# ebiggers/libdeflate

Measured on NVIDIA H100. Metric: MB/s compress+decompress (batched 64 KiB chunks), higher is better.
Workload: dtype u8

## Files before the change

### libdeflate_b200/csrc/deflate_kernel.cu

```cuda
#include "ldb_common.cuh"

#define DEF_THREADS 256

__global__ void __launch_bounds__(DEF_THREADS)
ldb_deflate_stored_kernel(ldb_deflate_args a)
{
	for (size_t c = blockIdx.x; c < a.n; c += gridDim.x) {
		const u8 *in = (const u8 *)a.in_ptrs[c];
		const size_t n = a.in_nbytes[c];
		u8 *out = (u8 *)a.out_ptrs[c];
		const size_t avail = a.out_avail[c];
		const u32 overhead = a.format == LDB_FMT_GZIP ? 18 : (a.format == LDB_FMT_ZLIB ? 6 : 0);
		const u32 hdr = a.format == LDB_FMT_GZIP ? 10 : (a.format == LDB_FMT_ZLIB ? 2 : 0);
		const size_t nblocks = n ? (n + 65534) / 65535 : 1;
		const size_t need = n + 5 * nblocks;
		bool fits = !(overhead && avail <= overhead) && need <= avail - overhead;
		if (!fits) {
			if (threadIdx.x == 0) a.out_nbytes[c] = 0;
			continue;
		}
		if (threadIdx.x == 0) def_write_header(out, a.format, a.level);
		const bool final_piece = !(a.piece && (a.piece[c] & LDB_PIECE_NONFINAL));
		u8 *dst = out + hdr;
		for (size_t b = 0; b < nblocks; b++) {
			size_t off = b * 65535;
			u32 len = (u32)(n - off > 65535 ? 65535 : n - off);
			if (threadIdx.x == 0) {
				dst[0] = (b + 1 == nblocks && final_piece) ? 1 : 0;
				dst[1] = (u8)len; dst[2] = (u8)(len >> 8);
				dst[3] = (u8)~len; dst[4] = (u8)(~len >> 8);
			}
			for (u32 i = threadIdx.x; i < len; i += DEF_THREADS) dst[5 + i] = in[off + i];
			dst += 5 + len;
		}
		if (threadIdx.x == 0) {
			u32 t = def_write_trailer(dst, a.format, a.checksums ? a.checksums[c] : 0, n);
			a.out_nbytes[c] = (size_t)(dst - out) + t;
		}
	}
}

#include "deflate_lz_kernel.cuh"

int ldb_deflate_grid(const ldb_launch_cfg &cfg) { return cfg.num_sms; }

int ldb_launch_deflate(const ldb_deflate_args &a, const ldb_launch_cfg &cfg, void *stream)
{
	if (a.n == 0) return 0;
	if (a.level == 0) {
		size_t blocks = a.n < (size_t)cfg.num_sms * 8 ? a.n : (size_t)cfg.num_sms * 8;
		LDB_LAUNCH(ldb_deflate_stored_kernel, dim3((unsigned)blocks), dim3(DEF_THREADS), 0, (cudaStream_t)stream, a);
		LDB_CUDA_CHECK_RET(cudaGetLastError());
		return 0;
	}
	return ldb_launch_deflate_lz(a, cfg, stream);
}
```

### libdeflate_b200/csrc/deflate_lz_kernel.cuh

```cuda
#pragma once

#ifndef LZ_THREADS
#define LZ_THREADS   1024
#endif
#define LZ_WARPS     (LZ_THREADS / 32)
#define LZ_PASS      16384
#define LZ_BLOCK_PASSES 2
#define LZ_NWIN      (LZ_PASS / 32)
#define LZ_NSL_BITS  (LZ_WARPS >= 32 ? 5 : 4)
#define LZ_NSL       (1 << LZ_NSL_BITS)
#ifndef LZ_QUANTUM
#define LZ_QUANTUM   0
#endif
#define LZ_SEG       16384
#define LZ_RING      65536
#define LZ_HASH_BITS 13
#define LZ_WIN       32768
#define LZ_LOOKAHEAD 512
#define LZ_MAX_DIST  (LZ_WIN - LZ_LOOKAHEAD)
#define LZ_TOKCAP    (LZ_BLOCK_PASSES * LZ_PASS + 64)
#define LZ_STAGE_WORDS 2048
#define LZ_TPT(gt)     ((gt) > 512 ? 1u : 2u)
#ifndef LZ_PWARPS
#define LZ_PWARPS    12
#endif
#define LZ_BAR_P     1
#ifndef LZ_PF
#define LZ_PF        4
#endif
#ifndef LZ_SPEC_ROUNDS
#define LZ_SPEC_ROUNDS 4
#endif
static_assert(LZ_SPEC_ROUNDS >= 1 && LZ_SPEC_ROUNDS <= 14, "round statistic buckets");
static_assert(LZ_PWARPS >= 10 && LZ_PWARPS < LZ_WARPS, "parse/flush group: 320..LZ_THREADS-32 threads");

#define LZ_SM_RING   0
#define LZ_SM_NEXT   (LZ_SM_RING + LZ_RING)
#define LZ_SM_HEAD   (LZ_SM_NEXT + 2 * 65536)
#define LZ_SM_R      (LZ_SM_HEAD + 2 * (1 << LZ_HASH_BITS))
#define LZ_SM_VIS    (LZ_SM_R)
#define LZ_SM_TOKOFF (LZ_SM_R + 4096)
#define LZ_SM_ENTRY  (LZ_SM_R + 8320)
#define LZ_SM_ESCAN  (LZ_SM_R + 9344)
#define LZ_SM_GEXIT  (LZ_SM_R + 9728)
#define LZ_SM_ITEMS  (LZ_SM_R + 12288)
#define LZ_SM_FREQ   (LZ_SM_ITEMS + 1024)
#define LZ_SM_LENS   (LZ_SM_FREQ + 4 * 320)
#define LZ_SM_CODES  (LZ_SM_LENS + 320)
#define LZ_SM_VARS   (LZ_SM_CODES + 2 * 320)
// ... 15 lines not shown
	u32 chunk;
	u32 tok_count;
	u32 parse_entry;
	u32 cost_dyn, cost_static, extra_bits;
	u32 hlit, hdist, hclen;
	u32 n_items;
	u32 run_counter;
	u32 min_len;
	u32 far4_dist;
	u32 used_lits[8];
	u32 carry;
	u32 nused_lit, nused_off;
	u32 huff_over;
	u32 obs_blk[8], obs_next[8];
	u32 end_early;
	u32 failed;
	u32 obit_lo, obit_hi;
	u32 blk_begin, blk_entry, blk_passes;
	u32 pre_lens_packed[3];
	u32 tma_phase;
	u32 dict, nonfinal;
	u32 spec_last;
	u32 spec_first;
};
static_assert(sizeof(lz_vars) <= 256, "lz_vars fits its shared-memory slot");

struct lz_params {
	int depth, nice, lazy;
	int opt_iters;
};

__device__ __forceinline__ lz_params lz_level_params(int level)
{
	switch (level) {
	case 1: return {2, 16, 0, 0};
	case 2: return {4, 24, 0, 0};
	case 3: return {8, 32, 0, 0};
	case 4: return {12, 48, 0, 0};
	case 5: return {12, 48, 1, 0};
#ifndef LZ_L6_DEPTH
#define LZ_L6_DEPTH 24
#endif
	case 6: return {LZ_L6_DEPTH, 96, 1, 0};
	case 7: return {48, 160, 1, 0};
	case 8: return {96, 258, 2, 0};
	case 9: return {200, 258, 2, 0};
// ... 10 lines not shown
	else if (num_used_literals < 8) m = 8;
	else if (num_used_literals < 10) m = 7;
	else if (num_used_literals < 16) m = 6;
	else if (num_used_literals < 45) m = 5;
	else m = 4;
	if (depth < 16) {
		u32 cap = depth < 5 ? 4 : (depth < 10 ? 5 : 7);
		if (m > cap) m = cap;
	}
	return m;
}

__device__ __forceinline__ u32 lz_ld32(const u8 *ring, u32 pos)
{
	u32 a = pos & (LZ_RING - 1);
	const u32 *w = (const u32 *)ring;
	u32 lo = w[a >> 2];
	u32 hi = w[((a + 4) & (LZ_RING - 1)) >> 2];
	return __funnelshift_r(lo, hi, (a & 3) * 8);
}
__device__ __forceinline__ u32 lz_ld8(const u8 *ring, u32 pos) { return ring[pos & (LZ_RING - 1)]; }
__device__ __forceinline__ u32 lz_hash(u32 v) { return (v * 0x1E35A7BDu) >> (32 - LZ_HASH_BITS); }

__device__ __forceinline__ void lz_load_segment(u8 *sm, lz_vars *v, const u8 *in, u32 from, u32 to)
{
	u8 *ring = sm + LZ_SM_RING;
	u32 len = to - from;
	u32 bulk = (((uintptr_t)(in + from) & 15) == 0) ? (len & ~15u) : 0;
	__syncthreads();
#ifndef LDB_EMU
	if (bulk) {
		u32 mbar = (u32)__cvta_generic_to_shared(&v->mbar);
		if (threadIdx.x == 0) {
			u32 dst = (u32)__cvta_generic_to_shared(ring + (from & (LZ_RING - 1)));
			asm volatile("fence.proxy.async.shared::cta;" ::: "memory");
			asm volatile("mbarrier.arrive.expect_tx.shared::cta.b64 _, [%0], %1;" ::"r"(mbar), "r"(bulk) : "memory");
			asm volatile("cp.async.bulk.shared::cluster.global.mbarrier::complete_tx::bytes [%0], [%1], %2, [%3];"
				     ::"r"(dst), "l"(in + from), "r"(bulk), "r"(mbar) : "memory");
		}
		u32 phase = v->tma_phase;
		u32 done = 0;
		while (!done) {
			asm volatile("{\n\t.reg .pred p;\n\tmbarrier.try_wait.parity.shared::cta.b64 p, [%1], %2;\n\tselp.u32 %0, 1, 0, p;\n\t}"
				     : "=r"(done) : "r"(mbar), "r"(phase) : "memory");
		}
	}
#else
	for (u32 i = threadIdx.x; i < bulk; i += LZ_THREADS) ring[(from + i) & (LZ_RING - 1)] = in[from + i];
#endif
	for (u32 i = bulk + threadIdx.x; i < len; i += LZ_THREADS) ring[(from + i) & (LZ_RING - 1)] = in[from + i];
	__syncthreads();
	if (bulk && threadIdx.x == 0) v->tma_phase ^= 1;
	__syncthreads();
}

__device__ __forceinline__ u32 lz_len_slot(u32 len)
{
	if (len < 11) return len - 3;
	if (len == 258) return 28;
	u32 l = len - 3;
	u32 eb = 29 - __clz(l);
	return 4 * eb + 4 + ((l >> eb) & 3);
}
__device__ __forceinline__ u32 lz_len_extra_bits(u32 slot) { return (slot < 8 || slot == 28) ? 0 : (slot - 4) >> 2; }
__device__ __forceinline__ u32 lz_len_base(u32 slot) { return slot < 8 ? 3 + slot : (slot == 28 ? 258 : 3 + ((4 + (slot & 3)) << ((slot - 4) >> 2))); }
__device__ __forceinline__ u32 lz_off_slot(u32 off)
{
	if (off < 5) return off - 1;
	u32 o = off - 1;
	u32 eb = 30 - __clz(o);
	return 2 * eb + 2 + ((o >> eb) & 1);
}
__device__ __forceinline__ u32 lz_off_extra_bits(u32 slot) { return slot < 4 ? 0 : (slot - 2) >> 1; }
__device__ __forceinline__ u32 lz_off_base(u32 slot) { return slot < 4 ? 1 + slot : 1 + ((2 + (slot & 1)) << ((slot - 2) >> 1)); }

__device__ __forceinline__ u32 lz_static_litlen_len(u32 sym) { return sym < 144 ? 8 : (sym < 256 ? 9 : (sym < 280 ? 7 : 8)); }
// ... 50 lines not shown
	}
}

__device__ __forceinline__ void lz_gen_codes_serial(const u8 *lens, u32 nsyms, u16 *codes)
{
	u32 cnt[16];
	for (u32 l = 0; l < 16; l++) cnt[l] = 0;
	for (u32 s = 0; s < nsyms; s++) cnt[lens[s]]++;
	u32 next[16];
	u32 code = 0;
	cnt[0] = 0;
	for (u32 l = 1; l < 16; l++) {
		next[l] = code;
		code = (code + cnt[l]) << 1;
	}
	for (u32 s = 0; s < nsyms; s++) {
		u32 l = lens[s];
		codes[s] = l ? (u16)(__brev(next[l]++) >> (32 - l)) : 0;
	}
}

#ifdef LZ_TIMING
#include <stdio.h>
__device__ unsigned long long ldb_lz_timing[2][16];
#define LZ_T(k) do { if (tid == 0 || tid == 32 * LZ_PWARPS) { long long t_ = clock64(); tacc[k] += t_ - tlast; tlast = t_; } } while (0)
#else
#define LZ_T(k) do { } while (0)
#endif

#ifdef LZ_SPEC_STATS
__device__ unsigned long long ldb_lz_spec_rounds[16];
extern "C" __attribute__((visibility("default"))) void ldb_lz_spec_stats(unsigned long long *out, int reset)
{
#ifdef LDB_EMU
	for (int i = 0; i < 16; i++) { out[i] = ldb_lz_spec_rounds[i]; if (reset) ldb_lz_spec_rounds[i] = 0; }
#else
	unsigned long long z[16] = {};
	cudaDeviceSynchronize();
	cudaMemcpyFromSymbol(out, ldb_lz_spec_rounds, sizeof(z));
	if (reset) cudaMemcpyToSymbol(ldb_lz_spec_rounds, z, sizeof(z));
#endif
}
#endif

template <int NBITS>
__device__ __forceinline__ u32 lz_same_key_mask(u32 key, bool valid)
{
	u32 m = __ballot_sync(LDB_FULL_MASK, valid);
#pragma unroll
	for (int b = 0; b < NBITS; b++) {
		const u32 bal = __ballot_sync(LDB_FULL_MASK, (key >> b) & 1);
		m &= ((key >> b) & 1) ? bal : ~bal;
	}
	return m;
}

__device__ __forceinline__ void lz_insert_pass_par(const u8 *ring, u16 *head, u16 *nextt, u32 *cmat,
						   u32 b0, u32 pend, u32 n, u32 tid, u32 lane, u32 warp
#ifdef LZ_TIMING
						   , long long *tacc, long long &tlast
#endif
						   )
{
	static_assert(LZ_WARPS >= LZ_NSL && (LZ_WARPS * LZ_NSL + 2 * LZ_NSL) * 4 <= 8192, "one linking warp per slice");
	u32 *sbase = cmat + LZ_WARPS * LZ_NSL, *stot = sbase + LZ_NSL;
	const u32 lt = (1u << lane) - 1;
	const u32 LB = (b0 + LZ_PASS) & 0xffff;
	const u32 ntiles = (pend - b0 + 31) >> 5, tpw = (ntiles + LZ_WARPS - 1) / LZ_WARPS;
	const u32 r0 = b0 + warp * tpw * 32;
	const u32 r1 = r0 + tpw * 32 < pend ? r0 + tpw * 32 : pend;
	for (u32 i = tid; i < LZ_WARPS * LZ_NSL + 2 * LZ_NSL; i += LZ_THREADS) cmat[i] = 0;
	__syncthreads();
	for (u32 p = r0 + lane; p < r1; p += 32) {
		const u32 hv = p + 4 <= n ? lz_hash(lz_ld32(ring, p)) : 0xffffu;
		nextt[p & 0xffff] = (u16)hv;
		if (hv != 0xffffu) atomicAdd(&cmat[warp * LZ_NSL + (hv >> (LZ_HASH_BITS - LZ_NSL_BITS))], 1u);
	}
	__syncthreads();
	LZ_T(12);
	if (warp == 0) {
		u32 run = 0;
		if (lane < LZ_NSL)
			for (u32 w = 0; w < LZ_WARPS; w++) {
				const u32 c = cmat[w * LZ_NSL + lane];
				cmat[w * LZ_NSL + lane] = run;
				run += c;
			}
		u32 incl = run;
		for (int o2 = 1; o2 < LZ_NSL; o2 <<= 1) {
			const u32 t = __shfl_up_sync(LDB_FULL_MASK, incl, o2);
			if (lane >= (u32)o2) incl += t;
		}
		if (lane < LZ_NSL) { sbase[lane] = incl - run; stot[lane] = run; }
	}
	__syncthreads();
	for (u32 t = 0; t < tpw; t++) {
		const u32 p = r0 + 32 * t + lane;
		const u32 hv = p < r1 ? nextt[p & 0xffff] : 0xffffu;
		const bool valid = hv != 0xffffu;
		const u32 sl = hv >> (LZ_HASH_BITS - LZ_NSL_BITS);
		const u32 m = lz_same_key_mask<LZ_NSL_BITS>(sl, valid);
		const u32 cur = valid ? cmat[warp * LZ_NSL + sl] : 0;
		__syncwarp();
		if (valid) {
			nextt[LB + sbase[sl] + cur + __popc(m & lt)] = (u16)p;
			if ((m & lt) == 0) cmat[warp * LZ_NSL + sl] = cur + __popc(m);
		}
		__syncwarp();
	}
	__syncthreads();
	LZ_T(13);
	if (warp < LZ_NSL) {
		const u32 cnt = stot[warp];
		const u16 *mylist = nextt + LB + sbase[warp];
		u32 p16n = lane < cnt ? mylist[lane] : 0;
		u32 hn = lane < cnt ? nextt[p16n] : 0;
		for (u32 b = 0; b < cnt; b += 32) {
			const bool valid = b + lane < cnt;
			const u32 p16 = p16n;
			const u32 h = valid ? hn : 0;
			if (b + 32 + lane < cnt) {
				p16n = mylist[b + 32 + lane];
				hn = nextt[p16n];
			}
			const u32 old_head = valid ? head[h] : 0;
			const u32 m = lz_same_key_mask<LZ_HASH_BITS - LZ_NSL_BITS>(h, valid);
			const u32 below = m & lt;
			const u32 prev = __shfl_sync(LDB_FULL_MASK, p16, below ? 31 - __clz(below) : 0);
			if (valid) {
				nextt[p16] = (u16)(below ? prev : old_head);
				if ((m >> lane) == 1) head[h] = (u16)p16;
			}
			__syncwarp();
		}
	}
	__syncthreads();
}

__device__ __forceinline__ void lz_search(const u8 *ring, const u16 *nextt, u32 p, u32 n, int depth, u32 nice_level,
					   u32 &best_len, u32 &best_dist)
{
	const u32 max_len = n - p < 258 ? n - p : 258;
	const u32 nice = nice_level < max_len ? nice_level : max_len;
	if (best_len) {
		while (best_len < max_len && lz_ld8(ring, p + best_len) == lz_ld8(ring, p - best_dist + best_len)) best_len++;
	}
	if (best_len >= nice) return;
	const u32 cur = lz_ld32(ring, p);
	u32 tailo = best_len >= 4 ? best_len - 3 : 0;
	u32 tailv = tailo ? lz_ld32(ring, p + tailo) : cur;
	const u32 lim = p < LZ_MAX_DIST ? p : LZ_MAX_DIST;
	u32 cand = nextt[p & 0xffff];
	u32 prev_dist = 0;
	for (int d = 0; d < depth; d++) {
		const u32 dist = (p - cand) & 0xffff;
		if (dist - 1 >= lim || dist <= prev_dist) break;
		prev_dist = dist;
		const u32 cq = cand;
		cand = nextt[cq];
// ... 244 lines not shown
	u32 *escan = (u32 *)(sm + LZ_SM_ESCAN);
	u16 *gexit = (u16 *)(sm + LZ_SM_GEXIT);
	u32 *freq = (u32 *)(sm + LZ_SM_FREQ);
	u8 *lens = sm + LZ_SM_LENS;
	u16 *codes = (u16 *)(sm + LZ_SM_CODES);
	lz_vars *v = (lz_vars *)(sm + LZ_SM_VARS);
	u32 *stage = (u32 *)(sm + LZ_SM_R);
	u16 *hsorted = (u16 *)(sm + LZ_SM_R);
	u32 *hnodefreq = (u32 *)(sm + LZ_SM_R + 1024);
	u16 *hparent = (u16 *)(sm + LZ_SM_R + 1024 + 2304);
	u16 *osorted = (u16 *)(sm + LZ_SM_R + 4608);
	u32 *onodefreq = (u32 *)(sm + LZ_SM_R + 4608 + 128);
	u16 *oparent = (u16 *)(sm + LZ_SM_R + 4608 + 128 + 512);
	u16 *items = (u16 *)(sm + LZ_SM_ITEMS);
	u8 *gs = a.scratch + 256 + (size_t)blockIdx.x * LZ_GS_BYTES;
	u32 *res = (u32 *)(gs + LZ_GS_RES);
	u32 *tokbuf = (u32 *)(gs + LZ_GS_TOK);
	u32 *costg = (u32 *)(gs + LZ_GS_COST);
	u32 *mlist = (u32 *)(gs + LZ_GS_MLIST);
	u8 *costtab = sm + LZ_SM_ITEMS;

	const u32 tid = threadIdx.x, lane = tid & 31, warp = tid >> 5;
#ifdef LZ_TIMING
	long long tacc[16] = {};
	long long tlast = clock64();
#endif
	const lz_params P = lz_level_params(a.level);
	const bool pipe = !P.opt_iters;
	u32 GW = LZ_WARPS, GT = LZ_THREADS;
	auto gsync = [&]() {
		if (GT < LZ_THREADS) LDB_BAR_SYNC(LZ_BAR_P, GT);
		else __syncthreads();
	};

	if (tid == 0) {
		v->tma_phase = 0;
#ifndef LDB_EMU
		u32 mbar = (u32)__cvta_generic_to_shared(&v->mbar);
		asm volatile("mbarrier.init.shared::cta.b64 [%0], 1;" ::"r"(mbar) : "memory");
		asm volatile("fence.mbarrier_init.release.cluster;" ::: "memory");
#endif
	}
	__syncthreads();

	for (;;) {
		if (tid == 0) v->chunk = atomicAdd(a.work_counter, 1u);
		__syncthreads();
		const size_t c = v->chunk;
		__syncthreads();
		if (c >= a.n) break;

		const u32 pflags = PIECES ? a.piece[c] : 0;
		const u32 dict = pflags & LDB_PIECE_DICT_MASK;
		const bool final_piece = !(pflags & LDB_PIECE_NONFINAL);
		const u8 *in = (const u8 *)a.in_ptrs[c];
		const size_t n64 = a.in_nbytes[c];
		lz_out o;
		o.out = (u8 *)a.out_ptrs[c];
		o.avail = a.out_avail[c];
		o.obit = 0;
		const u32 overhead = a.format == LDB_FMT_GZIP ? 18 : (a.format == LDB_FMT_ZLIB ? 6 : 0);
		const u32 trailer = a.format == LDB_FMT_GZIP ? 8 : (a.format == LDB_FMT_ZLIB ? 4 : 0);
		const u32 hdr_bytes = overhead - trailer;

		const bool passthrough = n64 <= (size_t)(55 - 4 * a.level) || n64 > 0x7fff0000u;
		bool fits = !(overhead && o.avail <= overhead);
		if (passthrough || !fits) {
			const size_t nblocks = n64 ? (n64 + 65534) / 65535 : 1;
			fits = fits && (n64 + 5 * nblocks <= o.avail - overhead);
			if (!fits) {
				if (tid == 0) a.out_nbytes[c] = 0;
				continue;
			}
			if (tid == 0) def_write_header(o.out, a.format, a.level);
			u8 *dst = o.out + hdr_bytes;
			for (size_t b = 0; b < nblocks; b++) {
				size_t off = b * 65535;
				u32 len = (u32)(n64 - off > 65535 ? 65535 : n64 - off);
				if (tid == 0) {
					dst[0] = (b + 1 == nblocks && final_piece) ? 1 : 0;
					dst[1] = (u8)len; dst[2] = (u8)(len >> 8);
					dst[3] = (u8)~len; dst[4] = (u8)(~len >> 8);
				}
				for (u32 i = tid; i < len; i += LZ_THREADS) dst[5 + i] = in[off + i];
				dst += 5 + len;
			}
			if (tid == 0) {
				u32 t = def_write_trailer(dst, a.format, a.checksums ? a.checksums[c] : 0, n64);
				a.out_nbytes[c] = (size_t)(dst - o.out) + t;
			}
			continue;
		}
		const u32 n = (u32)n64 + dict;
		in -= dict;

		for (u32 i = tid; i < (1u << LZ_HASH_BITS) / 2; i += LZ_THREADS) ((u32 *)head)[i] = 0xffffffffu;
		if (tid == 0) {
			v->failed = 0;
			v->parse_entry = dict;
			if (PIECES) { v->dict = dict; v->nonfinal = !final_piece; }
			v->tok_count = 0;
			u8 h[12] = {0, 0, 0, 0, 0, 0, 0, 0, 0, 0, 0, 0};
			def_write_header(h, a.format, a.level);
			u32 whole = hdr_bytes & ~3u;
			for (u32 i = 0; i < whole; i++) o.out[i] = h[i];
			u32 cw = 0;
			for (u32 i = whole; i < hdr_bytes; i++) cw |= (u32)h[i] << (8 * (i - whole));
			v->carry = cw;
		}
		for (u32 i = tid; i < 320; i += LZ_THREADS) freq[i] = 0;
		o.obit = (u64)hdr_bytes * 8;
		__syncthreads();

		auto parse_pass = [&](const u32 pb0, const u32 ppend, const u32 aoff, const bool forced, u16 *exitt) {
			const u32 nwin = (ppend - pb0 + 31) >> 5;
			const u32 min_len = v->min_len, far4 = v->far4_dist;
			const u32 G = (nwin + GW - 1) / GW;
			const u32 wbeg = warp * G, wend = wbeg + G < nwin ? wbeg + G : nwin;
			auto res_load = [&](u32 w) -> u32 {
				const u32 i = w * 32 + lane;
// ... 266 lines not shown
				for (u32 l = 15; l >= 1; l--) {
					cum += cn[l];
					if (myrank < cum) { len = l; break; }
				}
				lens[tid] = (u8)len;
			}
			gsync();
			if (tid < 320) {
				const u32 l = lens[tid];
				u32 code = 0;
				if (l) {
					const u32 *cn = is_lit ? hcount : ocount;
					u32 first = 0;
					for (u32 k = 1; k < l; k++) first = (first + cn[k]) << 1;
					u32 same = 0;
					for (u32 t = lo; t < tid; t++) same += lens[t] == l;
					code = __brev(first + same) >> (32 - l);
				}
				codes[tid] = (u16)code;
			}
			gsync();
		};

		u32 loaded_end = 0;
		u32 block_begin = dict;
		u32 block_entry = dict;
		u32 pass_in_block = 0;

		auto search_pass = [&](const u32 b0, const u32 pend, u32 *rs) {
			const u32 min_len = v->min_len, far4 = v->far4_dist;
#ifndef LZ_RUN_SHORT
#define LZ_RUN_SHORT 16
#endif
			const u32 run_len = a.level >= 7 ? 32 : LZ_RUN_SHORT;
			u32 i = 0, i_end = 0;
			u32 pL = 0, pD = 0;
			u32 pending = 0;
#if LZ_QUANTUM
			lz_walk wk;
			wk.left = 0; wk.best_len = 0; wk.best_dist = 0; wk.cand = 0; wk.prev_dist = 0; wk.tailo = 0; wk.tailv = 0; wk.cur = 0;
			bool in_search = false;
#endif
			for (;;) {
#if LZ_QUANTUM
				if (!in_search) {
#endif
				if (i >= i_end || b0 + i >= pend) {
					const u32 r = atomicAdd(&v->run_counter, 1u);
					i = r * run_len;
					if (b0 + i >= pend || i >= LZ_PASS) break;
					i_end = i + run_len;
					pending = 0;
				}
#if LZ_QUANTUM
					const u32 p0 = b0 + i;
					wk.best_len = 0; wk.best_dist = 0; wk.left = 0;
					if (p0 + 4 <= n) {
						u32 sL = 0, sD = 0;
						if (pending) { sL = pL - pending >= 4 ? pL - pending : 0; sD = pD; }
						lz_walk_setup(ring, nextt, p0, n, P.depth >> pending, (u32)P.nice, sL, sD, wk);
					}
					in_search = true;
				}
				lz_walk_steps(ring, nextt, b0 + i, n, (u32)P.nice, wk, LZ_QUANTUM);
				if (wk.left > 0) continue;
				in_search = false;
				const u32 p = b0 + i;
				u32 L = wk.best_len, D = wk.best_dist;
#else
				const u32 p = b0 + i;
				u32 L = 0, D = 0;
				if (p + 4 <= n) {
					if (pending) { L = pL - pending >= 4 ? pL - pending : 0; D = pD; }
					lz_search(ring, nextt, p, n, P.depth >> pending, (u32)P.nice, L, D);
				}
#endif
				rs[i] = L ? L | ((D - 1) << 16) : 0;
				u32 mpos, mL, mD;
				if (pending) {
					const int margin = pending == 1 ? 2 : 6;
					if (L >= pL && 4 * ((int)L - (int)pL) + ((int)(31 - __clz((int)pD)) - (int)(31 - __clz((int)D))) > margin) {
						mpos = i; mL = L >= (u32)P.nice ? L : 0; mD = D;
						if (!mL) { pL = L; pD = D; }
						pending = mL == 0 ? 1 : 0;
					} else if (pending == 1 && P.lazy == 2 && i + 1 < i_end && b0 + i + 1 < pend) {
						pending = 2;
						mpos = i; mL = 0; mD = 0;
					} else {
						mpos = i - pending; mL = pL; mD = pD;
						pending = 0;
					}
				} else if (L >= min_len && !(L == 4 && D > far4)) {
					if (P.lazy && L < (u32)P.nice && i + 1 < i_end && b0 + i + 1 < pend) {
						pending = 1; pL = L; pD = D;
						mpos = i; mL = 0; mD = 0;
					} else {
						mpos = i; mL = L; mD = D;
					}
				} else {
					mpos = i; mL = 0; mD = 0;
				}
				if (mL) {
					u32 stop = mpos + mL < i_end ? mpos + mL : i_end;
					if (b0 + stop > pend) stop = pend - b0;
					u32 mend = b0 + mpos + mL;
					for (u32 k = i + 1; k < stop; k++) {
						const u32 pk = b0 + k;
						if (mL == 258)
							while (mend < n && mend - pk < 258 && lz_ld8(ring, mend) == lz_ld8(ring, mend - mD)) mend++;
						u32 lk = mend - pk;
						rs[k] = lk >= 4 ? lk | ((mD - 1) << 16) : 0;
					}
					i = mpos + mL;
				} else {
					i++;
				}
			}
		};

		auto parse_and_flush = [&](const u32 b0, const u32 pend, const u32 aoff, u16 *exitt) {
			const bool last = pend >= n;
			parse_pass(b0, pend, aoff, false, exitt);
			LZ_T(2);
			pass_in_block++;
			if (!last) {
				if (tid < 8) v->obs_next[tid] = 0;
				gsync();
				lz_observe(ring, pend, pend + LZ_PASS < n ? pend + LZ_PASS : n, v->obs_next, tid, lane, GT);
				gsync();
				if (tid == 0) v->end_early = lz_should_end_block(v->obs_blk, v->obs_next, pend - block_begin) ? 1 : 0;
				gsync();
				const bool end_now = pass_in_block == LZ_BLOCK_PASSES || v->end_early;
// ... 385 lines not shown
						gsync();
						u32 carry = stage[full];
						gsync();
						for (u32 k = tid; k <= full && k < LZ_STAGE_WORDS; k += GT) stage[k] = 0;
						gsync();
						if (tid == 0) stage[0] = carry;
						w0 += full;
						rel &= 31;
						gsync();
					}
				}
				o.obit = (w0 << 5) + rel;
			}
			gsync();
			if (tid == 0) v->carry = stage[0];
			LZ_T(6);
			block_begin = block_end;
			block_entry = v->parse_entry;
			for (u32 i = tid; i < 320; i += GT) freq[i] = 0;
			if (tid == 0) v->tok_count = 0;
			gsync();
		};

		const u32 npass = (n + LZ_PASS - 1) / LZ_PASS;
		for (u32 step = 0; step < npass + (pipe ? 1 : 0); step++) {
			const u32 b0 = step * LZ_PASS;
			const u32 pend = b0 + LZ_PASS < n ? b0 + LZ_PASS : n;
			if (step < npass) {
				if (tid == 0) v->run_counter = 0;
				__syncthreads();
				{
					const u32 want = pend + LZ_PASS + 16 < n ? pend + LZ_PASS + 16 : n;
					while (loaded_end < want) {
						u32 room = LZ_RING - (loaded_end & (LZ_RING - 1));
						u32 to = loaded_end + (room < LZ_SEG ? room : LZ_SEG);
						if (to > want) to = want;
						lz_load_segment(sm, v, in, loaded_end, to);
						loaded_end = to;
					}
				}
				if (b0 == LZ_DICT) {
					if (tid < 8) { v->used_lits[tid] = 0; v->obs_blk[tid] = 0; }
					__syncthreads();
					lz_observe(ring, b0, pend, v->obs_blk, tid, lane, LZ_THREADS);
					const u32 own = n - LZ_DICT, scan = own < 4096 ? own : 4096;
					for (u32 i = tid; i < scan; i += LZ_THREADS) {
						u32 bv = ring[(b0 + i) & (LZ_RING - 1)];
						atomicOr(&v->used_lits[bv >> 5], 1u << (bv & 31));
					}
					__syncthreads();
					if (tid == 0) {
						u32 cnt = 0;
						for (int k = 0; k < 8; k++) cnt += __popc(v->used_lits[k]);
						v->min_len = own < 512 ? 4 : lz_choose_min_len(cnt, (u32)P.depth);
						v->far4_dist = cnt < 80 ? LZ_FAR4_DIST : LZ_WIN;
					}
					__syncthreads();
				}
				LZ_T(0);
#ifdef LZ_TIMING
				lz_insert_pass_par(ring, head, nextt, (u32 *)(sm + LZ_SM_R), b0, pend, n, tid, lane, warp, tacc, tlast);
#else
				lz_insert_pass_par(ring, head, nextt, (u32 *)(sm + LZ_SM_R), b0, pend, n, tid, lane, warp);
#endif
				LZ_T(3);
			}
			if (!pipe) {
				if (PIECES && step < v->dict / LZ_PASS) continue;
				u32 *rs = res + pass_in_block * LZ_PASS;
				for (u32 i = tid; b0 + i < pend; i += LZ_THREADS) {
					const u32 p = b0 + i;
					u32 L = 0, D = 0;
					u32 *ml = mlist + (size_t)(pass_in_block * LZ_PASS + i) * LZ_OPT_K;
					if (p + 4 <= n) {
						lz_search_all(ring, nextt, p, n, P.depth, (u32)P.nice, ml, L, D);
					} else {
						for (u32 k = 0; k < LZ_OPT_K; k++) ml[k] = 0;
					}
					rs[i] = L ? L | ((D - 1) << 16) : 0;
				}
				__syncthreads();
				LZ_T(1);
				parse_and_flush(b0, pend, pass_in_block * LZ_PASS, nextt + ((b0 + LZ_PASS) & 0xffff));
			} else {
				GW = step < npass ? LZ_PWARPS : LZ_WARPS;
				GT = 32 * GW;
				if (tid < GT && step > LZ_DICT / LZ_PASS) {
					const u32 kb0 = b0 - LZ_PASS;
					parse_and_flush(kb0, kb0 + LZ_PASS < n ? kb0 + LZ_PASS : n, ((step - 1) & 1) * LZ_PASS, nextt + ((kb0 + 2 * LZ_PASS) & 0xffff));
				}
				if (step < npass && (!PIECES || step >= v->dict / LZ_PASS)) search_pass(b0, pend, res + (step & 1) * LZ_PASS);
				LZ_T(1);
				if (tid == 0) {
					v->obit_lo = (u32)o.obit; v->obit_hi = (u32)(o.obit >> 32);
					v->blk_begin = block_begin; v->blk_entry = block_entry; v->blk_passes = pass_in_block;
				}
			}
			__syncthreads();
			LZ_T(14);
			if (v->failed) break;
			if (pipe) {
				o.obit = v->obit_lo | ((u64)v->obit_hi << 32);
				block_begin = v->blk_begin; block_entry = v->blk_entry; pass_in_block = v->blk_passes;
			}
		}
		__syncthreads();
		if (v->failed) {
			if (tid == 0) a.out_nbytes[c] = 0;
			__syncthreads();
			continue;
		}
		{
			u64 w0 = o.obit >> 5;
			for (u32 k = tid; k < LZ_STAGE_WORDS; k += LZ_THREADS) stage[k] = 0;
			__syncthreads();
			if (tid == 0) stage[0] = v->carry;
			__syncthreads();
			u64 ob;
			if (!LZ_NONFINAL) {
				ob = (o.obit + 7) & ~(u64)7;
				if (tid == 0 && trailer) {
					u8 t[8];
					def_write_trailer(t, a.format, a.checksums ? a.checksums[c] : 0, n64);
					for (u32 k = 0; k < trailer; k++) lz_stage_or(stage, (u32)(ob - (w0 << 5)) + 8 * k, t[k], 8);
				}
				ob += (u64)trailer * 8;
			} else {
				ob = (o.obit + 3 + 7) & ~(u64)7;
				if (tid == 0) lz_stage_or(stage, (u32)(ob - (w0 << 5)), 0xffff0000u, 32);
				ob += 32;
			}
			__syncthreads();
			u64 bytes_begin = w0 * 4, bytes_end = ob >> 3;
			for (u64 k = bytes_begin + tid; k < bytes_end; k += LZ_THREADS) {
				u32 rel = (u32)(k - bytes_begin);
				o.out[k] = (u8)(stage[rel >> 2] >> (8 * (rel & 3)));
			}
			if (tid == 0) a.out_nbytes[c] = (size_t)(ob >> 3);
		}
		__syncthreads();
		LZ_T(7);
	}
#ifdef LZ_TIMING
	if (tid == 0 || tid == 32 * LZ_PWARPS)
		for (int k = 0; k < 15; k++) atomicAdd(&ldb_lz_timing[tid != 0][k], (unsigned long long)tacc[k]);
#endif
}

#ifdef LZ_TIMING
extern "C" __attribute__((visibility("default"))) void ldb_lz_timing_dump(void)
{
	unsigned long long h[2][16], z[2][16] = {};
	cudaDeviceSynchronize();
	cudaMemcpyFromSymbol(h, ldb_lz_timing, sizeof(h));
	cudaMemcpyToSymbol(ldb_lz_timing, z, sizeof(z));
	const char *names[16] = {"loads+first", "search", "parse e5", "insert: linking", "huffman", "precode", "cost+emit", "chunk pro/epilogue",
				 "parse e1 steps", "parse e2 walks", "parse e3 exit", "parse e4", "insert: hashing", "insert: slice lists", "wait at join", ""};
	const char *who[2] = {"thread 0 (parse/flush group; levels 10-12: whole CTA)", "first thread of the search group"};
	for (int g = 0; g < 2; g++) {
		unsigned long long tot = 0;
		for (int k = 0; k < 15; k++) tot += h[g][k];
		printf("  timing, clocked by %s:\n", who[g]);
		for (int k = 0; k < 16; k++)
			if (h[g][k]) printf("  timing %-26s %14llu cycles  %5.1f%%\n", names[k], h[g][k], 100.0 * (double)h[g][k] / (double)tot);
	}
}
#endif

size_t ldb_deflate_scratch_bytes(const ldb_launch_cfg &cfg, size_t n)
{
	size_t ctas = n < (size_t)ldb_deflate_grid(cfg) ? n : (size_t)ldb_deflate_grid(cfg);
	return 256 + ctas * LZ_GS_BYTES;
}

static int ldb_launch_deflate_lz(const ldb_deflate_args &a, const ldb_launch_cfg &cfg, void *stream)
{
	LDB_CUDA_CHECK_RET(cudaFuncSetAttribute(a.piece ? ldb_deflate_lz_kernel<true> : ldb_deflate_lz_kernel<false>,
						cudaFuncAttributeMaxDynamicSharedMemorySize, LZ_SM_BYTES));
	ldb_deflate_args b = a;
	b.work_counter = (u32 *)a.scratch;
	LDB_CUDA_CHECK_RET(cudaMemsetAsync(b.work_counter, 0, sizeof(u32), (cudaStream_t)stream));
	size_t blocks = a.n < (size_t)ldb_deflate_grid(cfg) ? a.n : (size_t)ldb_deflate_grid(cfg);
	if (a.piece)
		LDB_LAUNCH(ldb_deflate_lz_kernel<true>, dim3((unsigned)blocks), dim3(LZ_THREADS), LZ_SM_BYTES, (cudaStream_t)stream, b);
	else
		LDB_LAUNCH(ldb_deflate_lz_kernel<false>, dim3((unsigned)blocks), dim3(LZ_THREADS), LZ_SM_BYTES, (cudaStream_t)stream, b);
// ... 4 lines not shown
```

### libdeflate_b200/csrc/ldb_common.cuh

```cuda
#pragma once

#include <stddef.h>
#include <stdint.h>

#ifndef LDB_EMU
#include <cuda_runtime.h>
#define LDB_DYN_SMEM(name) extern __shared__ __align__(128) uint8_t name[]
#define LDB_LAUNCH(kernel, grid, block, smem, stream, ...) \
	kernel<<<(grid), (block), (smem), (stream)>>>(__VA_ARGS__)
#define LDB_SPIN_PAUSE() __nanosleep(100)
#define LDB_BAR_SYNC(id, nthreads) asm volatile("bar.sync %0, %1;" ::"r"(id), "r"(nthreads) : "memory")
#else
#define LDB_SPIN_PAUSE() emu::yield()
static inline void ldb_emu_bar_sync(unsigned id, unsigned nthreads)
{
	static thread_local unsigned arrived[16], gen[16];
	if (id == 0 || id >= 16 || nthreads == 0 || nthreads % 32 || nthreads > emu::tl_block->nthreads) {
		fprintf(stderr, "bar.sync %u, %u is not a valid named barrier\n", id, nthreads);
		abort();
	}
	const unsigned mygen = gen[id];
	if (++arrived[id] == nthreads) {
		arrived[id] = 0;
		gen[id]++;
		emu::tl_block->spins = 0;
	} else {
		while (gen[id] == mygen) emu::yield();
	}
}
#define LDB_BAR_SYNC(id, nthreads) ldb_emu_bar_sync((id), (nthreads))
#endif

typedef uint8_t u8;
typedef uint16_t u16;
typedef uint32_t u32;
typedef uint64_t u64;
typedef int32_t s32;

#define LDB_FULL_MASK 0xffffffffu

#define LDB_SUCCESS            0
#define LDB_BAD_DATA           1
#define LDB_SHORT_OUTPUT       2
#define LDB_INSUFFICIENT_SPACE 3

#define LDB_FMT_RAW  0
#define LDB_FMT_ZLIB 1
#define LDB_FMT_GZIP 2

#define DEFLATE_BLOCKTYPE_STORED   0
#define DEFLATE_BLOCKTYPE_STATIC   1
#define DEFLATE_BLOCKTYPE_DYNAMIC  2
#define DEFLATE_NUM_PRECODE_SYMS   19
// ... 241 lines not shown
```

Before: 14910.

## Overlap next chunk's load, insert and first search with current chunk's final flush

In the pipelined LZ path, the CTA now claims its next chunk one pass early. During the last step, the search warps load that chunk's first segment, reset and build its hash chains, and run its first search pass, while the parse/flush warps finish and write out the current chunk. The next chunk's iteration then starts at step 1 with its min_len and far4 parameters already chosen. This hides per-chunk prologue latency (ring load, hash reset, insert) behind the epilogue, at the cost of named barriers, scratch-space aliasing for the count matrix, and a more complex control flow. An env var to cap the CTA count and extra timing spans are also added.

```diff
diff --git a/libdeflate_b200/csrc/deflate_kernel.cu b/libdeflate_b200/csrc/deflate_kernel.cu
--- a/libdeflate_b200/csrc/deflate_kernel.cu
+++ b/libdeflate_b200/csrc/deflate_kernel.cu
@@ -1,3 +1,5 @@
+#include <stdlib.h>
+
 #include "ldb_common.cuh"
 
 #define DEF_THREADS 256
@@ -42,7 +44,15 @@
 
 #include "deflate_lz_kernel.cuh"
 
-int ldb_deflate_grid(const ldb_launch_cfg &cfg) { return cfg.num_sms; }
+int ldb_deflate_grid(const ldb_launch_cfg &cfg)
+{
+	int g = cfg.num_sms;
+	if (const char *e = getenv("LIBDEFLATE_B200_DEFLATE_CTAS")) {
+		const int k = atoi(e);
+		if (k > 0 && k < g) g = k;
+	}
+	return g;
+}
 
 int ldb_launch_deflate(const ldb_deflate_args &a, const ldb_launch_cfg &cfg, void *stream)
 {
diff --git a/libdeflate_b200/csrc/deflate_lz_kernel.cuh b/libdeflate_b200/csrc/deflate_lz_kernel.cuh
--- a/libdeflate_b200/csrc/deflate_lz_kernel.cuh
+++ b/libdeflate_b200/csrc/deflate_lz_kernel.cuh
@@ -25,6 +25,8 @@
 #define LZ_PWARPS    12
 #endif
 #define LZ_BAR_P     1
+#define LZ_BAR_S     2
+#define LZ_BAR_H     3
 #ifndef LZ_PF
 #define LZ_PF        4
 #endif
@@ -86,6 +88,8 @@
 	u32 dict, nonfinal;
 	u32 spec_last;
 	u32 spec_first;
+	u32 prefetched;
+	u32 nx_min_len, nx_far4;
 };
 static_assert(sizeof(lz_vars) <= 256, "lz_vars fits its shared-memory slot");
 
@@ -142,16 +146,17 @@
 __device__ __forceinline__ u32 lz_ld8(const u8 *ring, u32 pos) { return ring[pos & (LZ_RING - 1)]; }
 __device__ __forceinline__ u32 lz_hash(u32 v) { return (v * 0x1E35A7BDu) >> (32 - LZ_HASH_BITS); }
 
-__device__ __forceinline__ void lz_load_segment(u8 *sm, lz_vars *v, const u8 *in, u32 from, u32 to)
+template <typename Bar>
+__device__ __forceinline__ void lz_load_segment(u8 *sm, lz_vars *v, const u8 *in, u32 from, u32 to, u32 gt, u32 gn, Bar bar)
 {
 	u8 *ring = sm + LZ_SM_RING;
 	u32 len = to - from;
 	u32 bulk = (((uintptr_t)(in + from) & 15) == 0) ? (len & ~15u) : 0;
-	__syncthreads();
+	bar();
 #ifndef LDB_EMU
 	if (bulk) {
 		u32 mbar = (u32)__cvta_generic_to_shared(&v->mbar);
-		if (threadIdx.x == 0) {
+		if (gt == 0) {
 			u32 dst = (u32)__cvta_generic_to_shared(ring + (from & (LZ_RING - 1)));
 			asm volatile("fence.proxy.async.shared::cta;" ::: "memory");
 			asm volatile("mbarrier.arrive.expect_tx.shared::cta.b64 _, [%0], %1;" ::"r"(mbar), "r"(bulk) : "memory");
@@ -166,12 +171,12 @@
 		}
 	}
 #else
-	for (u32 i = threadIdx.x; i < bulk; i += LZ_THREADS) ring[(from + i) & (LZ_RING - 1)] = in[from + i];
-#endif
-	for (u32 i = bulk + threadIdx.x; i < len; i += LZ_THREADS) ring[(from + i) & (LZ_RING - 1)] = in[from + i];
-	__syncthreads();
-	if (bulk && threadIdx.x == 0) v->tma_phase ^= 1;
-	__syncthreads();
+	for (u32 i = gt; i < bulk; i += gn) ring[(from + i) & (LZ_RING - 1)] = in[from + i];
+#endif
+	for (u32 i = bulk + gt; i < len; i += gn) ring[(from + i) & (LZ_RING - 1)] = in[from + i];
+	bar();
+	if (bulk && gt == 0) v->tma_phase ^= 1;
+	bar();
 }
 
 __device__ __forceinline__ u32 lz_len_slot(u32 len)
@@ -268,10 +273,14 @@
 
 #ifdef LZ_TIMING
 #include <stdio.h>
-__device__ unsigned long long ldb_lz_timing[2][16];
+__device__ unsigned long long ldb_lz_timing[2][18];
 #define LZ_T(k) do { if (tid == 0 || tid == 32 * LZ_PWARPS) { long long t_ = clock64(); tacc[k] += t_ - tlast; tlast = t_; } } while (0)
+#define LZ_TSPAN_BEGIN() do { if (tid == 0 || tid == 32 * LZ_PWARPS) tspan = clock64(); } while (0)
+#define LZ_TSPAN_END(k) do { if (tid == 0 || tid == 32 * LZ_PWARPS) tacc[k] += clock64() - tspan; } while (0)
 #else
 #define LZ_T(k) do { } while (0)
+#define LZ_TSPAN_BEGIN() do { } while (0)
+#define LZ_TSPAN_END(k) do { } while (0)
 #endif
 
 #ifdef LZ_SPEC_STATS
@@ -301,33 +310,34 @@
 	return m;
 }
 
+template <typename Bar>
 __device__ __forceinline__ void lz_insert_pass_par(const u8 *ring, u16 *head, u16 *nextt, u32 *cmat,
-						   u32 b0, u32 pend, u32 n, u32 tid, u32 lane, u32 warp
+						   u32 b0, u32 pend, u32 n, u32 tid, u32 lane, u32 warp, u32 gw, Bar bar
 #ifdef LZ_TIMING
 						   , long long *tacc, long long &tlast
 #endif
 						   )
 {
-	static_assert(LZ_WARPS >= LZ_NSL && (LZ_WARPS * LZ_NSL + 2 * LZ_NSL) * 4 <= 8192, "one linking warp per slice");
+	static_assert((LZ_WARPS * LZ_NSL + 2 * LZ_NSL) * 4 <= 8192, "count matrix fits the start of region R");
 	u32 *sbase = cmat + LZ_WARPS * LZ_NSL, *stot = sbase + LZ_NSL;
 	const u32 lt = (1u << lane) - 1;
 	const u32 LB = (b0 + LZ_PASS) & 0xffff;
-	const u32 ntiles = (pend - b0 + 31) >> 5, tpw = (ntiles + LZ_WARPS - 1) / LZ_WARPS;
+	const u32 ntiles = (pend - b0 + 31) >> 5, tpw = (ntiles + gw - 1) / gw;
 	const u32 r0 = b0 + warp * tpw * 32;
 	const u32 r1 = r0 + tpw * 32 < pend ? r0 + tpw * 32 : pend;
-	for (u32 i = tid; i < LZ_WARPS * LZ_NSL + 2 * LZ_NSL; i += LZ_THREADS) cmat[i] = 0;
-	__syncthreads();
+	for (u32 i = tid; i < LZ_WARPS * LZ_NSL + 2 * LZ_NSL; i += 32 * gw) cmat[i] = 0;
+	bar();
 	for (u32 p = r0 + lane; p < r1; p += 32) {
 		const u32 hv = p + 4 <= n ? lz_hash(lz_ld32(ring, p)) : 0xffffu;
 		nextt[p & 0xffff] = (u16)hv;
 		if (hv != 0xffffu) atomicAdd(&cmat[warp * LZ_NSL + (hv >> (LZ_HASH_BITS - LZ_NSL_BITS))], 1u);
 	}
-	__syncthreads();
+	bar();
 	LZ_T(12);
 	if (warp == 0) {
 		u32 run = 0;
 		if (lane < LZ_NSL)
-			for (u32 w = 0; w < LZ_WARPS; w++) {
+			for (u32 w = 0; w < gw; w++) {
 				const u32 c = cmat[w * LZ_NSL + lane];
 				cmat[w * LZ_NSL + lane] = run;
 				run += c;
@@ -339,7 +349,7 @@
 		}
 		if (lane < LZ_NSL) { sbase[lane] = incl - run; stot[lane] = run; }
 	}
-	__syncthreads();
+	bar();
 	for (u32 t = 0; t < tpw; t++) {
 		const u32 p = r0 + 32 * t + lane;
 		const u32 hv = p < r1 ? nextt[p & 0xffff] : 0xffffu;
@@ -354,11 +364,11 @@
 		}
 		__syncwarp();
 	}
-	__syncthreads();
+	bar();
 	LZ_T(13);
-	if (warp < LZ_NSL) {
-		const u32 cnt = stot[warp];
-		const u16 *mylist = nextt + LB + sbase[warp];
+	for (u32 s = warp; s < LZ_NSL; s += gw) {
+		const u32 cnt = stot[s];
+		const u16 *mylist = nextt + LB + sbase[s];
 		u32 p16n = lane < cnt ? mylist[lane] : 0;
 		u32 hn = lane < cnt ? nextt[p16n] : 0;
 		for (u32 b = 0; b < cnt; b += 32) {
@@ -380,7 +390,7 @@
 			__syncwarp();
 		}
 	}
-	__syncthreads();
+	bar();
 }
 
 __device__ __forceinline__ void lz_search(const u8 *ring, const u16 *nextt, u32 p, u32 n, int depth, u32 nice_level,
@@ -671,8 +681,8 @@
 
 	const u32 tid = threadIdx.x, lane = tid & 31, warp = tid >> 5;
 #ifdef LZ_TIMING
-	long long tacc[16] = {};
-	long long tlast = clock64();
+	long long tacc[18] = {};
+	long long tlast = clock64(), tspan = 0;
 #endif
 	const lz_params P = lz_level_params(a.level);
 	const bool pipe = !P.opt_iters;
@@ -684,6 +694,7 @@
 
 	if (tid == 0) {
 		v->tma_phase = 0;
+		v->prefetched = 0;
 #ifndef LDB_EMU
 		u32 mbar = (u32)__cvta_generic_to_shared(&v->mbar);
 		asm volatile("mbarrier.init.shared::cta.b64 [%0], 1;" ::"r"(mbar) : "memory");
@@ -693,10 +704,12 @@
 	__syncthreads();
 
 	for (;;) {
-		if (tid == 0) v->chunk = atomicAdd(a.work_counter, 1u);
+		if (tid == 0 && !v->prefetched) v->chunk = atomicAdd(a.work_counter, 1u);
 		__syncthreads();
 		const size_t c = v->chunk;
+		const bool pre = v->prefetched == 2;
 		__syncthreads();
+		if (tid == 0) v->prefetched = 0;
 		if (c >= a.n) break;
 
 		const u32 pflags = PIECES ? a.piece[c] : 0;
@@ -743,8 +756,8 @@
 		const u32 n = (u32)n64 + dict;
 		in -= dict;
 
-		for (u32 i = tid; i < (1u << LZ_HASH_BITS) / 2; i += LZ_THREADS) ((u32 *)head)[i] = 0xffffffffu;
 		if (tid == 0) {
+			if (pre) { v->min_len = v->nx_min_len; v->far4_dist = v->nx_far4; }
 			v->failed = 0;
 			v->parse_entry = dict;
 			if (PIECES) { v->dict = dict; v->nonfinal = !final_piece; }
@@ -1057,13 +1070,12 @@
 			gsync();
 		};
 
-		u32 loaded_end = 0;
+		u32 loaded_end = pre ? (n < 2 * LZ_PASS + 16 ? n : 2 * LZ_PASS + 16) : 0;
 		u32 block_begin = dict;
 		u32 block_entry = dict;
 		u32 pass_in_block = 0;
 
-		auto search_pass = [&](const u32 b0, const u32 pend, u32 *rs) {
-			const u32 min_len = v->min_len, far4 = v->far4_dist;
+		auto search_pass = [&](const u32 b0, const u32 pend, u32 *rs, const u32 nn, const u32 min_len, const u32 far4) {
 #ifndef LZ_RUN_SHORT
 #define LZ_RUN_SHORT 16
 #endif
@@ -1090,14 +1102,14 @@
 #if LZ_QUANTUM
 					const u32 p0 = b0 + i;
 					wk.best_len = 0; wk.best_dist = 0; wk.left = 0;
-					if (p0 + 4 <= n) {
+					if (p0 + 4 <= nn) {
 						u32 sL = 0, sD = 0;
 						if (pending) { sL = pL - pending >= 4 ? pL - pending : 0; sD = pD; }
-						lz_walk_setup(ring, nextt, p0, n, P.depth >> pending, (u32)P.nice, sL, sD, wk);
+						lz_walk_setup(ring, nextt, p0, nn, P.depth >> pending, (u32)P.nice, sL, sD, wk);
 					}
 					in_search = true;
 				}
-				lz_walk_steps(ring, nextt, b0 + i, n, (u32)P.nice, wk, LZ_QUANTUM);
+				lz_walk_steps(ring, nextt, b0 + i, nn, (u32)P.nice, wk, LZ_QUANTUM);
 				if (wk.left > 0) continue;
 				in_search = false;
 				const u32 p = b0 + i;
@@ -1105,9 +1117,9 @@
 #else
 				const u32 p = b0 + i;
 				u32 L = 0, D = 0;
-				if (p + 4 <= n) {
+				if (p + 4 <= nn) {
 					if (pending) { L = pL - pending >= 4 ? pL - pending : 0; D = pD; }
-					lz_search(ring, nextt, p, n, P.depth >> pending, (u32)P.nice, L, D);
+					lz_search(ring, nextt, p, nn, P.depth >> pending, (u32)P.nice, L, D);
 				}
 #endif
 				rs[i] = L ? L | ((D - 1) << 16) : 0;
@@ -1142,7 +1154,7 @@
 					for (u32 k = i + 1; k < stop; k++) {
 						const u32 pk = b0 + k;
 						if (mL == 258)
-							while (mend < n && mend - pk < 258 && lz_ld8(ring, mend) == lz_ld8(ring, mend - mD)) mend++;
+							while (mend < nn && mend - pk < 258 && lz_ld8(ring, mend) == lz_ld8(ring, mend - mD)) mend++;
 						u32 lk = mend - pk;
 						rs[k] = lk >= 4 ? lk | ((mD - 1) << 16) : 0;
 					}
@@ -1574,48 +1586,112 @@
 			gsync();
 		};
 
+		auto finish = [&]() {
+			if (v->failed) {
+				if (tid == 0) a.out_nbytes[c] = 0;
+				return;
+			}
+			u64 w0 = o.obit >> 5;
+			for (u32 k = tid; k < LZ_STAGE_WORDS; k += GT) stage[k] = 0;
+			gsync();
+			if (tid == 0) stage[0] = v->carry;
+			gsync();
+			u64 ob;
+			if (!LZ_NONFINAL) {
+				ob = (o.obit + 7) & ~(u64)7;
+				if (tid == 0 && trailer) {
+					u8 t[8];
+					def_write_trailer(t, a.format, a.checksums ? a.checksums[c] : 0, n64);
+					for (u32 k = 0; k < trailer; k++) lz_stage_or(stage, (u32)(ob - (w0 << 5)) + 8 * k, t[k], 8);
+				}
+				ob += (u64)trailer * 8;
+			} else {
+				ob = (o.obit + 3 + 7) & ~(u64)7;
+				if (tid == 0) lz_stage_or(stage, (u32)(ob - (w0 << 5)), 0xffff0000u, 32);
+				ob += 32;
+			}
+			gsync();
+			u64 bytes_begin = w0 * 4, bytes_end = ob >> 3;
+			for (u64 k = bytes_begin + tid; k < bytes_end; k += GT) {
+				u32 rel = (u32)(k - bytes_begin);
+				o.out[k] = (u8)(stage[rel >> 2] >> (8 * (rel & 3)));
+			}
+			if (tid == 0) a.out_nbytes[c] = (size_t)(ob >> 3);
+		};
+
 		const u32 npass = (n + LZ_PASS - 1) / LZ_PASS;
-		for (u32 step = 0; step < npass + (pipe ? 1 : 0); step++) {
+		const bool hand_on = pipe && !PIECES && (npass & 3) == 0;
+		bool handed = false;
+		for (u32 step = pre ? 1 : 0; step < npass + (pipe ? 1 : 0); step++) {
 			const u32 b0 = step * LZ_PASS;
 			const u32 pend = b0 + LZ_PASS < n ? b0 + LZ_PASS : n;
-			if (step < npass) {
-				if (tid == 0) v->run_counter = 0;
-				__syncthreads();
+			LZ_TSPAN_BEGIN();
+			size_t c1 = 0;
+			u32 n1 = 0;
+			bool beside = false;
+			if (hand_on && step == npass) {
+				c1 = v->chunk;
+				if (c1 < a.n) {
+					const size_t m64 = a.in_nbytes[c1];
+					n1 = (u32)m64;
+					beside = !(m64 <= (size_t)(55 - 4 * a.level) || m64 > 0x7fff0000u) && !(overhead && a.out_avail[c1] <= overhead);
+				}
+			}
+			const bool sg = beside && warp >= LZ_PWARPS;
+			if (step < npass || sg) {
+				const u32 gt = sg ? tid - 32 * LZ_PWARPS : tid, gw = sg ? LZ_WARPS - LZ_PWARPS : LZ_WARPS, gn = 32 * gw;
+				auto gbar = [&]() {
+					if (sg) LDB_BAR_SYNC(LZ_BAR_S, LZ_THREADS - 32 * LZ_PWARPS);
+					else __syncthreads();
+				};
+				const u8 *src = sg ? (const u8 *)a.in_ptrs[c1] : in;
+				const u32 fn = sg ? n1 : n, fb0 = sg ? 0 : b0, fpend = sg ? (n1 < LZ_PASS ? n1 : LZ_PASS) : pend;
+				if (sg) loaded_end = 0;
+				if (gt == 0) {
+					v->run_counter = 0;
+					if (hand_on && step + 1 == npass) { v->chunk = atomicAdd(a.work_counter, 1u); v->prefetched = 1; }
+				}
+				if (fb0 == 0)
+					for (u32 i = gt; i < (1u << LZ_HASH_BITS) / 2; i += gn) ((u32 *)head)[i] = 0xffffffffu;
+				gbar();
 				{
-					const u32 want = pend + LZ_PASS + 16 < n ? pend + LZ_PASS + 16 : n;
+					const u32 want = fpend + LZ_PASS + 16 < fn ? fpend + LZ_PASS + 16 : fn;
 					while (loaded_end < want) {
 						u32 room = LZ_RING - (loaded_end & (LZ_RING - 1));
 						u32 to = loaded_end + (room < LZ_SEG ? room : LZ_SEG);
 						if (to > want) to = want;
-						lz_load_segment(sm, v, in, loaded_end, to);
+						lz_load_segment(sm, v, src, loaded_end, to, gt, gn, gbar);
 						loaded_end = to;
 					}
 				}
-				if (b0 == LZ_DICT) {
-					if (tid < 8) { v->used_lits[tid] = 0; v->obs_blk[tid] = 0; }
-					__syncthreads();
-					lz_observe(ring, b0, pend, v->obs_blk, tid, lane, LZ_THREADS);
-					const u32 own = n - LZ_DICT, scan = own < 4096 ? own : 4096;
-					for (u32 i = tid; i < scan; i += LZ_THREADS) {
-						u32 bv = ring[(b0 + i) & (LZ_RING - 1)];
+				if (fb0 == LZ_DICT) {
+					if (gt < 8) { v->used_lits[gt] = 0; v->obs_blk[gt] = 0; }
+					gbar();
+					lz_observe(ring, fb0, fpend, v->obs_blk, gt, lane, gn);
+					const u32 own = fn - LZ_DICT, scan = own < 4096 ? own : 4096;
+					for (u32 i = gt; i < scan; i += gn) {
+						u32 bv = ring[(fb0 + i) & (LZ_RING - 1)];
 						atomicOr(&v->used_lits[bv >> 5], 1u << (bv & 31));
 					}
-					__syncthreads();
-					if (tid == 0) {
+					gbar();
+					if (gt == 0) {
 						u32 cnt = 0;
 						for (int k = 0; k < 8; k++) cnt += __popc(v->used_lits[k]);
-						v->min_len = own < 512 ? 4 : lz_choose_min_len(cnt, (u32)P.depth);
-						v->far4_dist = cnt < 80 ? LZ_FAR4_DIST : LZ_WIN;
-					}
-					__syncthreads();
+						(sg ? v->nx_min_len : v->min_len) = own < 512 ? 4 : lz_choose_min_len(cnt, (u32)P.depth);
+						(sg ? v->nx_far4 : v->far4_dist) = cnt < 80 ? LZ_FAR4_DIST : LZ_WIN;
+					}
+					gbar();
 				}
 				LZ_T(0);
+				u32 *cmat = sg ? (u32 *)(nextt + 2 * LZ_PASS) : (u32 *)(sm + LZ_SM_R);
 #ifdef LZ_TIMING
-				lz_insert_pass_par(ring, head, nextt, (u32 *)(sm + LZ_SM_R), b0, pend, n, tid, lane, warp, tacc, tlast);
+				lz_insert_pass_par(ring, head, nextt, cmat, fb0, fpend, fn, gt, lane, warp - (sg ? LZ_PWARPS : 0), gw, gbar, tacc, tlast);
 #else
-				lz_insert_pass_par(ring, head, nextt, (u32 *)(sm + LZ_SM_R), b0, pend, n, tid, lane, warp);
+				lz_insert_pass_par(ring, head, nextt, cmat, fb0, fpend, fn, gt, lane, warp - (sg ? LZ_PWARPS : 0), gw, gbar);
 #endif
 				LZ_T(3);
+				if (step == 0) LZ_TSPAN_END(17);
+				if (sg) LDB_BAR_ARRIVE(LZ_BAR_H, LZ_THREADS);
 			}
 			if (!pipe) {
 				if (PIECES && step < v->dict / LZ_PASS) continue;
@@ -1635,85 +1711,67 @@
 				LZ_T(1);
 				parse_and_flush(b0, pend, pass_in_block * LZ_PASS, nextt + ((b0 + LZ_PASS) & 0xffff));
 			} else {
-				GW = step < npass ? LZ_PWARPS : LZ_WARPS;
+				GW = step < npass || beside ? LZ_PWARPS : LZ_WARPS;
 				GT = 32 * GW;
 				if (tid < GT && step > LZ_DICT / LZ_PASS) {
 					const u32 kb0 = b0 - LZ_PASS;
-					parse_and_flush(kb0, kb0 + LZ_PASS < n ? kb0 + LZ_PASS : n, ((step - 1) & 1) * LZ_PASS, nextt + ((kb0 + 2 * LZ_PASS) & 0xffff));
-				}
-				if (step < npass && (!PIECES || step >= v->dict / LZ_PASS)) search_pass(b0, pend, res + (step & 1) * LZ_PASS);
+					parse_and_flush(kb0, kb0 + LZ_PASS < n ? kb0 + LZ_PASS : n, ((step - 1) & 1) * LZ_PASS,
+							nextt + ((kb0 + (beside ? 0 : 2 * LZ_PASS)) & 0xffff));
+					if (beside) {
+						finish();
+						LDB_BAR_SYNC(LZ_BAR_H, LZ_THREADS);
+					}
+				}
+				if ((step < npass && (!PIECES || step >= v->dict / LZ_PASS)) || beside)
+					search_pass(beside ? 0 : b0, beside ? (n1 < LZ_PASS ? n1 : LZ_PASS) : pend, res + (beside ? 0 : (step & 1) * LZ_PASS),
+						    beside ? n1 : n, beside ? v->nx_min_len : v->min_len, beside ? v->nx_far4 : v->far4_dist);
 				LZ_T(1);
 				if (tid == 0) {
 					v->obit_lo = (u32)o.obit; v->obit_hi = (u32)(o.obit >> 32);
 					v->blk_begin = block_begin; v->blk_entry = block_entry; v->blk_passes = pass_in_block;
 				}
+				if (beside && tid == 32 * LZ_PWARPS) v->prefetched = 2;
 			}
 			__syncthreads();
 			LZ_T(14);
+			if (step == npass) LZ_TSPAN_END(16);
+			if (beside) { handed = true; break; }
 			if (v->failed) break;
 			if (pipe) {
 				o.obit = v->obit_lo | ((u64)v->obit_hi << 32);
 				block_begin = v->blk_begin; block_entry = v->blk_entry; pass_in_block = v->blk_passes;
 			}
 		}
+		if (handed) continue;
 		__syncthreads();
-		if (v->failed) {
-			if (tid == 0) a.out_nbytes[c] = 0;
-			__syncthreads();
-			continue;
-		}
-		{
-			u64 w0 = o.obit >> 5;
-			for (u32 k = tid; k < LZ_STAGE_WORDS; k += LZ_THREADS) stage[k] = 0;
-			__syncthreads();
-			if (tid == 0) stage[0] = v->carry;
-			__syncthreads();
-			u64 ob;
-			if (!LZ_NONFINAL) {
-				ob = (o.obit + 7) & ~(u64)7;
-				if (tid == 0 && trailer) {
-					u8 t[8];
-					def_write_trailer(t, a.format, a.checksums ? a.checksums[c] : 0, n64);
-					for (u32 k = 0; k < trailer; k++) lz_stage_or(stage, (u32)(ob - (w0 << 5)) + 8 * k, t[k], 8);
-				}
-				ob += (u64)trailer * 8;
-			} else {
-				ob = (o.obit + 3 + 7) & ~(u64)7;
-				if (tid == 0) lz_stage_or(stage, (u32)(ob - (w0 << 5)), 0xffff0000u, 32);
-				ob += 32;
-			}
-			__syncthreads();
-			u64 bytes_begin = w0 * 4, bytes_end = ob >> 3;
-			for (u64 k = bytes_begin + tid; k < bytes_end; k += LZ_THREADS) {
-				u32 rel = (u32)(k - bytes_begin);
-				o.out[k] = (u8)(stage[rel >> 2] >> (8 * (rel & 3)));
-			}
-			if (tid == 0) a.out_nbytes[c] = (size_t)(ob >> 3);
-		}
+		GW = LZ_WARPS;
+		GT = LZ_THREADS;
+		finish();
 		__syncthreads();
 		LZ_T(7);
 	}
 #ifdef LZ_TIMING
 	if (tid == 0 || tid == 32 * LZ_PWARPS)
-		for (int k = 0; k < 15; k++) atomicAdd(&ldb_lz_timing[tid != 0][k], (unsigned long long)tacc[k]);
+		for (int k = 0; k < 18; k++) atomicAdd(&ldb_lz_timing[tid != 0][k], (unsigned long long)tacc[k]);
 #endif
 }
 
 #ifdef LZ_TIMING
 extern "C" __attribute__((visibility("default"))) void ldb_lz_timing_dump(void)
 {
-	unsigned long long h[2][16], z[2][16] = {};
+	unsigned long long h[2][18], z[2][18] = {};
 	cudaDeviceSynchronize();
 	cudaMemcpyFromSymbol(h, ldb_lz_timing, sizeof(h));
 	cudaMemcpyToSymbol(ldb_lz_timing, z, sizeof(z));
-	const char *names[16] = {"loads+first", "search", "parse e5", "insert: linking", "huffman", "precode", "cost+emit", "chunk pro/epilogue",
-				 "parse e1 steps", "parse e2 walks", "parse e3 exit", "parse e4", "insert: hashing", "insert: slice lists", "wait at join", ""};
+	const char *names[18] = {"loads+first", "search", "parse e5", "insert: linking", "huffman", "precode", "cost+emit", "chunk pro/epilogue",
+				 "parse e1 steps", "parse e2 walks", "parse e3 exit", "parse e4", "insert: hashing", "insert: slice lists", "wait at join", "",
+				 "(span) last step", "(span) step 0 load+insert"};
 	const char *who[2] = {"thread 0 (parse/flush group; levels 10-12: whole CTA)", "first thread of the search group"};
 	for (int g = 0; g < 2; g++) {
 		unsigned long long tot = 0;
 		for (int k = 0; k < 15; k++) tot += h[g][k];
 		printf("  timing, clocked by %s:\n", who[g]);
-		for (int k = 0; k < 16; k++)
+		for (int k = 0; k < 18; k++)
 			if (h[g][k]) printf("  timing %-26s %14llu cycles  %5.1f%%\n", names[k], h[g][k], 100.0 * (double)h[g][k] / (double)tot);
 	}
 }
diff --git a/libdeflate_b200/csrc/ldb_common.cuh b/libdeflate_b200/csrc/ldb_common.cuh
--- a/libdeflate_b200/csrc/ldb_common.cuh
+++ b/libdeflate_b200/csrc/ldb_common.cuh
@@ -10,9 +10,10 @@
 	kernel<<<(grid), (block), (smem), (stream)>>>(__VA_ARGS__)
 #define LDB_SPIN_PAUSE() __nanosleep(100)
 #define LDB_BAR_SYNC(id, nthreads) asm volatile("bar.sync %0, %1;" ::"r"(id), "r"(nthreads) : "memory")
+#define LDB_BAR_ARRIVE(id, nthreads) asm volatile("bar.arrive %0, %1;" ::"r"(id), "r"(nthreads) : "memory")
 #else
 #define LDB_SPIN_PAUSE() emu::yield()
-static inline void ldb_emu_bar_sync(unsigned id, unsigned nthreads)
+static inline void ldb_emu_bar_sync(unsigned id, unsigned nthreads, bool wait = true)
 {
 	static thread_local unsigned arrived[16], gen[16];
 	if (id == 0 || id >= 16 || nthreads == 0 || nthreads % 32 || nthreads > emu::tl_block->nthreads) {
@@ -24,11 +25,12 @@
 		arrived[id] = 0;
 		gen[id]++;
 		emu::tl_block->spins = 0;
-	} else {
+	} else if (wait) {
 		while (gen[id] == mygen) emu::yield();
 	}
 }
 #define LDB_BAR_SYNC(id, nthreads) ldb_emu_bar_sync((id), (nthreads))
+#define LDB_BAR_ARRIVE(id, nthreads) ldb_emu_bar_sync((id), (nthreads), false)
 #endif
 
 typedef uint8_t u8;
```

Result: faster. 15560 (median of 6 runs) (+4.4%).
